# labgem/pangenomeNEM

Hardware: AMD Instinct MI355X
Metric: em_family_x_organism_cells_per_sec (higher is better)
Workload: dtype f32 chains with f64 intermediates (reference arithmetic); int32 popcounts in the M-step; 1 GPU; BASELINE configs[1]: 20000 families x 500 organisms, K=3, beta=0.5, contiguity graph (path + 5% chords, weights 1..8), ncem/sk_/pk; U-shaped family-frequency spectrum (Beta(0.3, 0.3) per family), default .m init; families_total=20000, families_per_gpu=20000, organisms=500, K=3, parallelism=1 GPU

## Files before the change

### pangenomenem_amd/csrc/nem_engine.hip

```cpp
#include <hip/hip_runtime.h>
#include <dlfcn.h>
#include <pthread.h>
#include <unistd.h>

#include <algorithm>
#include <atomic>
#include <cfloat>
#include <chrono>
#include <cmath>
#include <cstdio>
#include <cstdlib>
#include <cstring>
#include <condition_variable>
#include <deque>
#include <functional>
#include <map>
#include <string>
#include <mutex>
#include <thread>
#include <vector>

#include "nem_internal.hpp"
#include "nem_ff.hpp"
#include "nem_chain.hpp"
// ... 59 lines not shown
    void* rccl_comm = nullptr;
    int sh_world = 1, sh_rank = 0, sh_blk = 0, sh_stride = 0;
    const uint8_t* shard_lab[3] = {nullptr, nullptr, nullptr};
    int sh_tot_off() const { return ((sh_blk + 3) & ~3) + 4; }
    int npad = 0, dpad = 0, W = 0, wf = 0, nw64 = 0, device = 0;
    hipStream_t stream = nullptr;
    bool own_stream = false;
    nemgpu_config cfg{};
    bool have_matrix = false, have_params = false, has_graph = false;
    bool reset_pending = false;

    uint32_t* xw = nullptr;
    uint32_t* xws = nullptr;
    int* perm = nullptr;
    uint32_t* host_bits = nullptr; size_t host_bits_words = 0, host_bits_pin = 0;
    std::vector<uint32_t> host_bits_own;
    struct Staged { char* p; size_t size; };
    std::vector<Staged> staging;
    bool use_sort = true;
    uint64_t* xt = nullptr;
    int *nei_ptr = nullptr, *nei_idx = nullptr;
    float* nei_w = nullptr;
    int nnz = 0;

    float *prop = nullptr, *center = nullptr, *disp = nullptr;
    float *prop0 = nullptr, *center0 = nullptr, *disp0 = nullptr;
    size_t par_o_center = 0, par_o_disp = 0, par_o_nb = 0, par_words = 0;
    float *nbobs_k = nullptr, *iner = nullptr;
    int *fz_lastz = nullptr, *fz_any1 = nullptr;
    float *fz_in0 = nullptr, *fz_in1 = nullptr, *fz_inh = nullptr;
    float* fz_ct = nullptr;
    float* fz_chk = nullptr;
    double2* tabT = nullptr;
    double* tabL0 = nullptr;
    uint32_t *nz0 = nullptr, *nz1 = nullptr, *am0 = nullptr, *am1 = nullptr;
    double2* uni = nullptr;
    int* nonuni = nullptr;
    uint2* ffq = nullptr;
    int* sweep_next = nullptr;
    bool tables_fresh = false;
    bool density_fresh = false;
    double* pk = nullptr;
    float* logpk = nullptr;
    double* pkfki = nullptr;
    float* logpkfki = nullptr;

// ... 502 lines not shown

int do_density(nemgpu_engine* e)
{
    launch_density(finish_args(e, 0, nullptr), e->xws, e->n, e->npad, e->pkfki, e->logpkfki, e->iter_flags() + FLAG_MOVED,
                   kSweepFlagWords, e->stream);
    HIPCHK(hipGetLastError());
    e->flags_clean = true;
    e->density_fresh = true;
    return NEMGPU_OK;
}

struct SweepCtx {
    SweepArgs a{};
    bool use_nei = false;
    bool multi = false;
    int r = 0;
    int checked = 0;
    int slot_base = 0;
    bool post = false; bool post_moved = false; CtrlArgs post_ctrl{};
    SweepArgs* hold = nullptr;
    int* count_into = nullptr;
};

int clear_sweep_flags(nemgpu_engine* e)
{
    if (current_recorder()) launch_fill(e->iter_flags() + FLAG_MOVED, kSweepFlagWords, 0, e->stream);
    else HIPCHK(hipMemsetAsync(e->iter_flags() + FLAG_MOVED, 0, kSweepFlagWords * sizeof(int), e->stream));
    e->flags_clean = true;
    return NEMGPU_OK;
}

int ensure_draw_window(nemgpu_engine* e, long lo, long count)
{
    if (e->draw_valid && e->draw_tab0 <= lo && lo + count <= e->draw_tab0 + e->draw_cap) return NEMGPU_OK;
    if (e->draw_borrowed) {
        e->draw_borrowed = false; e->draw_valid = false; e->draw_tab = nullptr; e->draw_cap = 0;
    }
    long cap = std::max<long>(e->draw_cap, 1024);
    while (cap < 2 * count) cap *= 2;
    if (!e->draw_valid || lo < e->draw_tab0) {
        e->draw_gen.seed(e->cfg.tie_seed); e->draw_gen_pos = 0; e->draw_host.clear(); e->draw_tab0 = 0;
    }
    const long have_end = e->draw_tab0 + (long)e->draw_host.size();
    if (lo >= have_end) {
        while (e->draw_gen_pos < lo) { (void)e->draw_gen.next(); e->draw_gen_pos++; }
        e->draw_host.clear();
// ... 76 lines not shown
                continue;
            }
        } else if (c.post && ncem && r0 == 0 && b == count - 1) {
            c.a.post_on = 1; c.a.post_from_guess = (r % 2 == 1) ? 1 : 0; c.a.post_moved = c.post_moved ? 1 : 0;
            c.a.post_skip_guess = c.a.post_from_guess;
            c.a.post_nw64 = e->nw64; c.a.post_mask = e->mask; c.a.post_flags = e->iter_flags(); c.a.post_ctrl = c.post_ctrl;
        }
        launch_sweep(c.a, ncem, e->stream);
    }
    HIPCHK(hipGetLastError());
    return NEMGPU_OK;
}

int sweep_setup(nemgpu_engine* e, float beta, SweepCtx& c, bool id_by_value)
{
    c.use_nei = e->has_graph && beta != 0.0f;
    c.multi = c.use_nei || e->libc();
    SweepArgs& a = c.a;
    a.n_local = e->n; a.lo = e->lo; a.n_total = e->n_total; a.K = e->k; a.npad = e->npad;
    a.use_nei = c.use_nei ? 1 : 0;
    a.nei_ptr = e->nei_ptr; a.nei_idx = e->nei_idx; a.nei_w = e->nei_w;
    a.beta = beta;
    a.pkfki = e->pkfki;
    a.tie_rule = e->cfg.tie_rule; a.tie_seed = e->cfg.tie_seed; a.sweep_id = e->sweep_counter++;
    a.sweep_id_ptr = (e->stop_ptr != nullptr && !id_by_value) ? e->sweep_next : nullptr;
    if (e->libc()) {
        if (e->stop_ptr == nullptr) { int r = ensure_draw_window(e, e->draws, draw_need(e)); if (r) return r; }
        sweep_draw_args(e, a, e->stop_ptr == nullptr);
    }
    return NEMGPU_OK;
}

int sweep_enqueue(nemgpu_engine* e, float beta, SweepCtx& c, bool id_by_value = false, const CtrlArgs* post_ctrl = nullptr,
                  bool post_moved = false, int slot_base = 0, int rounds = 0, SweepArgs* hold = nullptr, int* count_into = nullptr)
{
    c = SweepCtx();
    c.slot_base = slot_base;
    if (post_ctrl != nullptr && e->ncem()) {
        c.post = true; c.post_moved = post_moved; c.post_ctrl = *post_ctrl; c.hold = hold;
        c.count_into = hold != nullptr ? count_into : nullptr;
    }
    { int r = sweep_setup(e, beta, c, id_by_value); if (r) return r; }
    if (!e->flags_clean) { int r = clear_sweep_flags(e); if (r) return r; }
    e->flags_clean = false;
    return sweep_launch_rounds(e, c, c.multi ? (rounds > 0 ? rounds : e->round_batch) : 1);
}
// ... 119 lines not shown
    if (e->ncem()) return do_labels_post(e, newbuf, oldbuf, ctrl);
    if (e->cfg.cvtest == NEMGPU_CV_CLAS) {
        launch_conv_fuzzy((size_t)e->n * e->k, e->cbuf[newbuf] + (size_t)e->lo * e->k,
                          e->cbuf[oldbuf] + (size_t)e->lo * e->k, e->cfg.cvthres, e->iter_flags(), e->stop_ptr, ctrl,
                          e->stream);
        HIPCHK(hipGetLastError());
    } else if (ctrl != nullptr) {
        launch_ctrl(*ctrl, e->stream);
        HIPCHK(hipGetLastError());
    }
    return NEMGPU_OK;
}

constexpr int kPipeDepth = 7;

int host_rounds_ctx(nemgpu_engine* e, SweepCtx& sc, uint32_t sweep_id, int launched)
{
    sc = SweepCtx();
    sc.use_nei = e->has_graph && e->cfg.beta != 0.0f;
    sc.multi = true;
    SweepArgs& a = sc.a;
    a.n_local = e->n; a.lo = e->lo; a.n_total = e->n_total; a.K = e->k; a.npad = e->npad; a.use_nei = sc.use_nei ? 1 : 0;
    a.nei_ptr = e->nei_ptr; a.nei_idx = e->nei_idx; a.nei_w = e->nei_w; a.beta = e->cfg.beta; a.pkfki = e->pkfki;
    a.tie_rule = e->cfg.tie_rule; a.tie_seed = e->cfg.tie_seed; a.sweep_id = sweep_id; a.sweep_id_ptr = nullptr;
    sc.r = launched; sc.checked = launched;
    if (e->libc()) {
        for (int q = 0; q < launched; q++) if (e->h_round(q)[FLAG_NTIES] & (1 << 30)) e->tie_heavy = true;
        int r = ensure_draw_window(e, e->draws, draw_need(e));
        if (r) return r;
        sweep_draw_args(e, a, true);
    }
    return NEMGPU_OK;
}

int iteration_rounds(const nemgpu_engine* e, int pos, bool deep)
{
    int want = (current_recorder() != nullptr || deep || !e->ncem()) ? e->round_batch : e->rounds_iter;
    if (!e->ncem() && current_recorder() == nullptr && pos >= 0 && pos < kFzPositions && e->fz_need[pos] > want) want = e->fz_need[pos];
    return want;
}

int enqueue_iteration(nemgpu_engine* e, int cur, uint32_t sweep_id, bool defer_ctrl, bool deep, int pos = -1)
{
    int r;
    const int saved = e->cur;
    e->cur = cur;
// ... 1285 lines not shown
    HIPCHK(hipSetDevice(device));
    nemgpu_engine* e = new nemgpu_engine();
    e->n_total = n_total; e->n_true = n_total; e->d = d; e->k = k; e->lo = site_lo; e->hi = site_hi; e->n = site_hi - site_lo;
    e->device = device;
    e->npad = (e->n + 255) / 256 * 256;
    e->dpad = (d + 63) / 64 * 64;
    e->W = e->dpad / 32;
    e->wf = (d + 31) / 32;
    e->nw64 = (e->n + 63) / 64;
    e->cfg.algo = NEMGPU_ALGO_NCEM; e->cfg.beta = 0.5f; e->cfg.disper = NEMGPU_DISP_K_; e->cfg.propor = NEMGPU_PROP_K;
    e->cfg.cvtest = NEMGPU_CV_CLAS; e->cfg.cvthres = 1e-8f; e->cfg.it_max = 100; e->cfg.param_fix = 0;
    e->cfg.tie_rule = NEMGPU_TIE_HASH; e->cfg.tie_seed = 0;
    if (const char* g = getenv("NEM_MI355X_GRAPHS")) e->use_graphs = (g[0] != '0');
    if (const char* g = getenv("NEM_MI355X_SHADOW_VERIFY")) e->shadow_verify = (g[0] != '0');
    e->flag_sets = e->shadow_verify ? 3 : 1;
    if (const char* g = getenv("NEM_MI355X_ROUND_COUNTS")) e->round_counts = (g[0] != '0');
    if (const char* g = getenv("NEM_MI355X_START_FUSED")) e->start_fused = (g[0] != '0');
    if (const char* g = getenv("NEM_MI355X_ROUNDS")) e->round_batch = std::max(2, std::min(kRoundBatchMax, atoi(g)));
    if (const char* g = getenv("NEM_MI355X_ROUNDS_ITER")) e->rounds_iter = std::max(2, std::min(e->round_batch, atoi(g)));
    e->rounds_iter = std::min(e->rounds_iter, e->round_batch);
    if (const char* g = getenv("NEM_MI355X_FAULT_INJECT")) e->fault_inject = !strcmp(g, "fuzzy_pc") ? 1 : 0;
    if (const char* g = getenv("NEM_MI355X_FF")) e->ff_mode = (g[0] == '0') ? 0 : (g[0] == '1') ? 1 : -1;
    if (const char* g = getenv("NEM_MI355X_SORT")) e->use_sort = (g[0] != '0');
    if (hip_stream) { e->stream = (hipStream_t)hip_stream; e->own_stream = false; }
    else {
        if (pool_stream_get(device, &e->stream) != hipSuccess) { delete e; set_error("hipStreamCreate failed"); return NEMGPU_E_DEVICE; }
        e->own_stream = true;
    }
    int r = NEMGPU_OK;
    alloc_for(e);
    auto A = [&](int rr) { if (r == NEMGPU_OK) r = rr; };
    A(dev_alloc(&e->xw, (size_t)e->W * e->npad));
    A(dev_alloc(&e->xws, (size_t)((e->W + 3) / 4) * 4 * e->npad));
    A(dev_alloc(&e->perm, (size_t)e->npad));
    A(dev_alloc(&e->xt, (size_t)d * e->nw64));
    A(alloc_model_buffers(e));
    if (r == NEMGPU_OK && !e->flags_host &&
        pool_get(device, true, e->flag_words() * sizeof(int), (char**)&e->flags_host, &e->flags_host_size) != hipSuccess) {
        set_error("hipHostMalloc failed"); r = NEMGPU_E_DEVICE;
    }
    if (r != NEMGPU_OK) { nemgpu_destroy(e); return r; }
    e->draw_ctl = e->sweep_next + 8;
    *out = e;
    return NEMGPU_OK;
}

// ... 233 lines not shown
    {
        std::vector<std::thread> th;
        for (int t = 1; t < nt; t++)
            th.emplace_back(pack_rows, (int)((long long)e->n * t / nt), (int)((long long)e->n * (t + 1) / nt), &badv[t]);
        pack_rows(0, (int)((long long)e->n / nt), &badv[0]);
        for (std::thread& x : th) x.join();
    }
    g_packers.fetch_sub(1);
    const uint64_t bad = badv[0] | badv[1] | badv[2] | badv[3];
    if (bad & 0xFEFEFEFEFEFEFEFEull) { e->host_bits_words = 0; set_error("presence/absence matrix must hold 0/1 only"); return NEMGPU_E_ARG; }
    return upload_bits(e, pc.data());
}

int nemgpu_set_graph(nemgpu_engine* e, const int32_t* ptr, const int32_t* idx, const float* w)
{
    if (!e || !ptr) return NEMGPU_E_FUNCARG;
    HIPCHK(hipSetDevice(e->device));
    const int nnz = ptr[e->n] - ptr[0];
    if (ptr[0] != 0 || nnz < 0) { set_error("graph: ptr[0] must be 0 and ptr non-decreasing"); return NEMGPU_E_ARG; }
    for (int i = 0; i < e->n; i++) if (ptr[i + 1] < ptr[i]) { set_error("graph: ptr not monotone"); return NEMGPU_E_ARG; }
    for (int t = 0; t < nnz; t++)
        if (idx[t] < 0 || idx[t] >= e->n_total) { set_error("graph: neighbour index out of range"); return NEMGPU_E_ARG; }
    e->nei_ptr = nullptr; e->nei_idx = nullptr; e->nei_w = nullptr;
    int r;
    alloc_for(e);
    const size_t b_ptr = sizeof(int) * ((size_t)e->n + 1), b_nz = sizeof(int) * (size_t)nnz;
    const size_t o_idx = (b_ptr + 255) & ~(size_t)255, o_w = (o_idx + b_nz + 255) & ~(size_t)255, total = o_w + b_nz;
    char* dev = nullptr;
    if ((r = dev_alloc(&dev, total))) return r;
    e->nei_ptr = (int*)dev; e->nei_idx = (int*)(dev + o_idx); e->nei_w = (float*)(dev + o_w);
    char* st = stage(e, total);
    if (st) {
        memcpy(st, ptr, b_ptr);
        if (nnz > 0) { memcpy(st + o_idx, idx, b_nz); memcpy(st + o_w, w, b_nz); }
        HIPCHK(hipMemcpyAsync(dev, st, total, hipMemcpyHostToDevice, e->stream));
    } else {
        HIPCHK(hipMemcpyAsync(e->nei_ptr, ptr, b_ptr, hipMemcpyHostToDevice, e->stream));
        if (nnz > 0) {
            HIPCHK(hipMemcpyAsync(e->nei_idx, idx, b_nz, hipMemcpyHostToDevice, e->stream));
            HIPCHK(hipMemcpyAsync(e->nei_w, w, b_nz, hipMemcpyHostToDevice, e->stream));
        }
        HIPCHK(hipStreamSynchronize(e->stream));
    }
    e->nnz = nnz;
    e->has_graph = nnz > 0;
    drop_graphs(e);
    return NEMGPU_OK;
}

int nemgpu_set_params(nemgpu_engine* e, const float* prop, const float* center, const float* disp)
{
    if (!e || !prop || !center || !disp) return NEMGPU_E_FUNCARG;
    HIPCHK(hipSetDevice(e->device));
    const size_t kd = (size_t)e->k * e->d;
    float* st = e->parent == nullptr ? (float*)stage(e, sizeof(float) * e->par_words) : nullptr;
    if (st) {
        memset(st, 0, sizeof(float) * e->par_words);
        memcpy(st, prop, sizeof(float) * e->k); memcpy(st + e->par_o_center, center, sizeof(float) * kd);
        memcpy(st + e->par_o_disp, disp, sizeof(float) * kd);
        HIPCHK(hipMemcpyAsync(e->prop0, st, sizeof(float) * e->par_words, hipMemcpyHostToDevice, e->stream));
    } else {
        HIPCHK(copy_sync(e, e->prop0, prop, sizeof(float) * e->k, hipMemcpyHostToDevice));
        HIPCHK(copy_sync(e, e->center0, center, sizeof(float) * kd, hipMemcpyHostToDevice));
        HIPCHK(copy_sync(e, e->disp0, disp, sizeof(float) * kd, hipMemcpyHostToDevice));
    }
    e->have_params = true;
    return reset_state(e, true);
}

int nemgpu_configure(nemgpu_engine* e, const nemgpu_config* cfg)
// ... 843 lines not shown
    if (m->block) (void)hipFree(m->block);
    delete m;
}

static int adopt_chunk(nemgpu_engine* e, const nemgpu_master* M, const nemk::ChunkPlan& plan, int nnz_c)
{
    if (e->device != M->device) { set_error("a chunk's engine lives on its master's device"); return NEMGPU_E_ARG; }
    HIPCHK(hipSetDevice(e->device));
    alloc_for(e);
    int r;
    const size_t words = (size_t)e->n * e->wf;
    if ((r = dev_alloc(&e->xf_stage, words + (size_t)e->npad))) return r;
    e->perm = reinterpret_cast<int*>(e->xf_stage + words);
    const int nnz = std::max(nnz_c, 0);
    const size_t b_ptr = sizeof(int) * ((size_t)e->n + 1), b_nz = sizeof(int) * (size_t)std::max(nnz, 1);
    const size_t o_idx = (b_ptr + 255) & ~(size_t)255, o_w = (o_idx + b_nz + 255) & ~(size_t)255, total = o_w + b_nz;
    char* dev = nullptr;
    if ((r = dev_alloc(&dev, total))) return r;
    e->nei_ptr = (int*)dev; e->nei_idx = (int*)(dev + o_idx); e->nei_w = (float*)(dev + o_w);
    nemk::ChunkFill f{e->n, e->d, e->wf, e->npad, e->xf_stage, e->perm, e->nei_ptr, e->nei_idx, e->nei_w};
    nemk::launch_chunk_fill(M->dev, plan, f, e->stream);
    HIPCHK(hipGetLastError());
    e->nnz = nnz; e->has_graph = nnz > 0;
    e->host_bits = nullptr; e->host_bits_words = 0;
    if (e->defer_layout) e->layout_pending = true;
    else { launch_layout(e->xf_stage, e->n, e->wf, e->W, e->npad, e->d, e->nw64, e->xw, e->xt, e->perm, e->xws, e->stream); HIPCHK(hipGetLastError()); }
    e->have_matrix = true;
    return NEMGPU_OK;
}

static int solve_chunks_impl(nemgpu_master* M, nemgpu_chunk* chunks, int count, int k, const float* prop, const float* center_k,
                             const float* disp_k, const nemgpu_config* cfg, int workers, int group, nemgpu_votes* votes,
                             ResampleTally* tally = nullptr)
{
    if (!M || !chunks || count <= 0 || k <= 0 || k > kMaxKernelK || !prop || !center_k || !disp_k || !cfg) return NEMGPU_E_FUNCARG;
    HIPCHK(hipSetDevice(M->device));
    const int n = M->n, nw64 = M->nw64, wf = M->wf, nnz = M->nnz;
    size_t org_total = 0;
    int max_dc = 0;
    for (int c = 0; c < count; c++) {
        nemgpu_chunk& q = chunks[c];
        q.rc = NEMGPU_OK; q.n = 0; q.nnz = 0; q.result = nemgpu_result{};
        if (!q.organisms || q.dc <= 0 || q.dc > M->d) { set_error("nemgpu_solve_chunks: chunk " + std::to_string(c) + ": 1 .. d organisms are needed"); return NEMGPU_E_FUNCARG; }
        for (int t = 0; t < q.dc; t++)
            if (q.organisms[t] < 0 || q.organisms[t] >= M->d) { set_error("nemgpu_solve_chunks: chunk " + std::to_string(c) + ": organism index out of range"); return NEMGPU_E_ARG; }
        org_total += ((size_t)q.dc + 63) & ~(size_t)63;
// ... 592 lines not shown
        e->masks_valid = false; e->tables_fresh = false; e->density_fresh = false;
        if ((r = do_mstep(e)) || (!e->ncem() && (r = read_iter_flags(e)))) { cleanup(); return r; }
        e->status = NEMGPU_OK; e->emptyk = 0;
        e->iters = best_res.iters; e->converged = best_res.converged;
        if (res) { *res = best_res; res->status = NEMGPU_OK; res->tie_draws = e->draws; for (int t = 0; t < 6; t++) res->crit[t] = best_crit[t]; }
    } else if (res) {
        fill_result(e, res);
        res->status = last_status;
    }
    if (best_start) *best_start = best;
    cleanup();
    return NEMGPU_OK;
}

static int make_clone(nemgpu_engine* p, nemgpu_engine** out, char* slab, size_t slab_bytes, int* flags_host, float* par0)
{
    nemgpu_engine* c = new nemgpu_engine();
    c->n_total = p->n_total; c->n_true = p->n_true; c->d = p->d; c->k = p->k; c->lo = p->lo; c->hi = p->hi; c->n = p->n;
    c->npad = p->npad; c->dpad = p->dpad; c->W = p->W; c->wf = p->wf; c->nw64 = p->nw64; c->device = p->device;
    c->stream = p->stream; c->own_stream = false;
    c->cfg = p->cfg; c->have_matrix = true; c->have_params = true; c->has_graph = p->has_graph;
    c->xw = p->xw; c->xws = p->xws; c->perm = p->perm; c->xt = p->xt; c->use_sort = p->use_sort;
    c->nei_ptr = p->nei_ptr; c->nei_idx = p->nei_idx; c->nei_w = p->nei_w; c->nnz = p->nnz;
    c->use_graphs = p->use_graphs; c->ff_mode = p->ff_mode; c->round_batch = p->round_batch; c->rounds_iter = p->rounds_iter;
    c->parent = p; c->carve_all = true;
    c->chunks.push_back({slab, slab_bytes, 0, false});
    c->shared_chunk = 0;
    c->flags_host = flags_host; c->flags_host_borrowed = true;
    const size_t kd = (size_t)p->k * p->d;
    c->prop0 = par0; c->center0 = par0 + p->k; c->disp0 = par0 + p->k + kd;
    alloc_for(c);
    int r = alloc_model_buffers(c);
    if (r == NEMGPU_OK) r = ensure_state_buffers(c);
    if (r == NEMGPU_OK) r = ensure_crit_buffers(c);
    alloc_for(p);
    if (r != NEMGPU_OK) { nemgpu_destroy(c); return r; }
    c->draw_ctl = c->sweep_next + 8;
    *out = c;
    return NEMGPU_OK;
}

static int ensure_clones(nemgpu_engine* e, int count)
{
    if ((int)e->clones.size() >= count) return NEMGPU_OK;
    HIPCHK(hipStreamSynchronize(e->stream));
    for (nemgpu_engine* c : e->clones) nemgpu_destroy(c);
// ... 351 lines not shown

int nemgpu_stats_words(const nemgpu_engine* e) { return e ? e->k + e->k * e->d : 0; }

int nemgpu_shard_layout(nemgpu_engine* e, int world, int rank, int blk, int stride, int n_true)
{
    if (!e || world <= 0 || rank < 0 || rank >= world || blk <= 0 || stride < blk + 1 || n_true <= 0) return NEMGPU_E_FUNCARG;
    if (e->lo != rank * stride || e->n > blk || e->n_total != world * stride) {
        set_error("shard layout does not match the engine's slot range");
        return NEMGPU_E_ARG;
    }
    if (stride % 4 != 0) { set_error("shard layout: stride must be a multiple of 4 bytes"); return NEMGPU_E_ARG; }
    e->sh_world = world; e->sh_rank = rank; e->sh_blk = blk; e->sh_stride = stride; e->n_true = n_true;
    return NEMGPU_OK;
}

namespace {
void shard_sweep_args(nemgpu_engine* e, SweepArgs& a, float beta, int sweep_id)
{
    a = SweepArgs{};
    a.n_local = e->n; a.lo = e->lo; a.n_total = e->n_total; a.K = e->k; a.npad = e->npad;
    a.use_nei = (e->has_graph && beta != 0.0f) ? 1 : 0;
    a.nei_ptr = e->nei_ptr; a.nei_idx = e->nei_idx; a.nei_w = e->nei_w;
    a.beta = beta; a.pkfki = e->pkfki;
    a.tie_rule = e->cfg.tie_rule; a.tie_seed = e->cfg.tie_seed;
    a.sweep_id = sweep_id >= 0 ? (uint32_t)sweep_id : 0u;
    a.sweep_id_ptr = sweep_id >= 0 ? nullptr : e->sweep_next;
    a.stop = e->stop_ptr;
    a.n_ranks = e->sh_world; a.slot_stride = e->sh_stride; a.slot_pad = e->sh_stride - e->sh_blk;
    a.fold_ticket = e->sweep_next + 32;
    if (e->libc()) { sweep_draw_args(e, a, e->stop_ptr == nullptr); a.rank_index = e->sh_rank; }
}
uint8_t* own_flag_byte(nemgpu_engine* e, uint8_t* labels) { return labels + (size_t)e->sh_rank * e->sh_stride + e->sh_blk; }
int shard_buf(const nemgpu_engine* e, const uint8_t* p) { for (int b = 0; b < 3; b++) if (e->shard_lab[b] == p) return b; return -1; }
int shard_tie_args(nemgpu_engine* e, SweepArgs& a, const uint8_t* guess, uint8_t* out)
{
    if (!e->libc()) return NEMGPU_OK;
    const int g = shard_buf(e, guess), o = shard_buf(e, out);
    if (g < 0 || o < 0) { set_error("TIE_LIBC in the sharded path: a label array that nemgpu_shard_set_labels was not told about"); return NEMGPU_E_FUNCARG; }
    a.tie_cnt_guess = e->tie_cnt[g]; a.tie_cnt_out = e->tie_cnt[o];
    a.rank_tot_in = guess + e->sh_tot_off();
    a.rank_tot_out = out + (size_t)e->sh_rank * e->sh_stride + e->sh_tot_off();
    return NEMGPU_OK;
}
void shard_round1_args(nemgpu_engine* e, SweepArgs& a, float beta, int sweep_id, const uint8_t* labels_old_dev,
                       const uint8_t* labels_guess_dev, uint8_t* labels_out_dev)
{
// ... 974 lines not shown
```

### pangenomenem_amd/csrc/nem_kernels.hpp

```cpp
#pragma once
#include <hip/hip_runtime.h>
#include <cstdint>
#include <cstring>
#include <type_traits>
#include <vector>

#include "../../include/nem_mi355x.h"

namespace nemk {

constexpr int kMaxKernelK = 32;
constexpr int kTicketWords = 32 * 33;
constexpr double kEpsilonD = 1e-20;

enum { FLAG_CHANGED = 0, FLAG_NZERO = 1, FLAG_FIRSTZERO = 2, FLAG_NTIES = 3, FLAG_ROUND_STRIDE = 4 };
enum { FLAG_EMPTYK = 0, FLAG_EMPTY_PROP = 1, FLAG_FAULT = 2, FLAG_MOVED = 3, FLAG_ITER_STRIDE = 4 };

enum { C_STOP = 0, C_FOLD = 1, C_ITERS = 10, C_COMMITS = 2, C_STATUS = 3, C_EMPTYK = 4, C_CONVERGED = 5, C_NEED_ROUNDS = 6,
       C_SWEEP_ROUNDS = 7, C_NZERO = 8, C_FIRSTZERO = 9, C_DRAWS = 11, C_DEEP = 12, C_DRAWS_INIT = 13, C_INIT_ROUNDS = 14, C_WORDS = 16 };

struct CtrlArgs {
    int* ctrl; const int* iter_flags; const int* round0;
    int n_rounds;
    int param_fix, use_nei, cvtest, ncem; float cvthres;
// ... 14 lines not shown
    const int* nei_ptr; const int* nei_idx; const float* nei_w;
    float beta;
    const double* pkfki;
    const uint8_t* lab_old; const uint8_t* lab_guess; uint8_t* lab_out;
    const float* c_old; const float* c_guess; float* c_out;
    int tie_rule; uint32_t tie_seed; uint32_t sweep_id;
    const int* sweep_id_ptr;
    int* flags;
    const int* prev_changed;
    const int* stop;
    const uint8_t* flags_in; int n_ranks, slot_stride, slot_pad;
    int post_on, post_from_guess, post_moved, post_nw64, post_skip_guess;
    int post_no_masks;
    uint64_t* post_mask; int* post_flags;
    CtrlArgs post_ctrl;
    uint8_t* publish_byte; int* publish_ticket;
    int* fold_ticket;
    const uint32_t* draw_tab; int draw_tab_len, draw_base, draw_tab0;
    const int* draw_ctl; const int* draw_extra;
    const int* tie_cnt_guess; int* tie_cnt_out;
    const uint8_t* rank_tot_in; int rank_index; uint8_t* rank_tot_out;
    int spb;
    int* post_stats; const uint64_t* post_xt; int post_D;
};
struct LabelsPostArgs { int n_local, lo, K, nw64; const uint8_t* lab_new; const uint8_t* lab_old; uint64_t* mask; int* flags;
                        const int* stop; CtrlArgs ca; };
struct CountsArgs { int K, D, nw64; const uint64_t* xt; const uint64_t* mask; int* stats; const int* stop; CtrlArgs prev_ctrl; };
struct FuzzyArgs { int n, npad, K, D; const uint32_t* xw; const uint64_t* xt; int nw64; const float* c; float* nbobs_k;
                   float* in0; float* in1; float* inh_k; int* lastz; int* any1; float* center; float* iner; const int* stop;
                   float* ct; int ctpad;
                   float* chk;
                   int* fault;
                   int inject; };
struct ConvFuzzyArgs { size_t m; const float* c; const float* cold; float thres; int* flags; const int* stop; CtrlArgs ca; };
struct OnehotArgs { int n, K; const uint8_t* lab; float* c; };
struct CritArgs { int n, K, npad; const int* nei_ptr; const int* nei_idx; const float* nei_w; int use_nei; float beta;
                  const float* c; const double* pkfki; const float* logpkfki; float* dik; float* gik; double* lfi; double* lzi;
                  float* crit6; int hard; };
struct FillArgs { int* ptr; int words; int value; };
struct CopyArgs { const int* src; int* dst; int words; };
struct CopySegsArgs { const int* src[8]; int* dst[8]; int words[8]; int n; };
void launch_copy_segments(const CopySegsArgs& a, hipStream_t s);
struct LayoutArgs { const uint32_t* xf; const int* perm; int n, wf, W, npad, d, nw64; uint32_t* xw; uint32_t* xws; uint64_t* xt; };

enum OpKind { OP_FINISH = 1, OP_DENSITY, OP_DENSITY_FUSED, OP_SWEEP, OP_COUNTS, OP_LABELS_POST, OP_CTRL,
              OP_CONV_FUZZY, OP_ONEHOT, OP_CRIT_TERMS, OP_CRIT_REDUCE, OP_CRIT_FINAL, OP_FILL, OP_COPY, OP_FUZZY_T,
              OP_FUZZY_PC, OP_FUZZY_MED2, OP_LAYOUT_WORDS, OP_LAYOUT_BITS };
// ... 91 lines not shown
```

### pangenomenem_amd/csrc/nem_sweep.hip

```cpp
#include <hip/hip_runtime.h>
#include <algorithm>
#include <cstdio>
#include <cstdlib>

#include "nem_kernels.hpp"
#include "nem_sweep_dev.hpp"

namespace nemk {

template <int KT, bool NCEM, int BS, bool LIBC = false, bool COUNT = false>
__global__ __launch_bounds__(BS) void k_sweep(SweepArgs a) { sweep_body<KT, NCEM, BS, LIBC, COUNT>(a, blockIdx.x, gridDim.x); }
template <int KT, bool NCEM, int BS, bool LIBC = false>
__global__ __launch_bounds__(BS) void k_sweep_b(const void* arr, int stride, const int* gx) { NEM_B_HEAD(SweepArgs) sweep_body<KT, NCEM, BS, LIBC>(a, blockIdx.x, nblk); }

static int sweep_variant(int K, bool ncem, bool big, bool libc) { return (K >= 1 && K <= 10 ? K : 0) | (ncem ? 16 : 0) | (big ? 32 : 0) | (libc && ncem ? 64 : 0); }

template <bool BATCHED>
static void sweep_dispatch(int variant, dim3 grid, unsigned bdim, hipStream_t s, const SweepArgs* a, const void* arr, int stride, const int* gx)
{
    const int kt = variant & 15; const bool ncem = (variant & 16) != 0, big = (variant & 32) != 0, libc = (variant & 64) != 0;
    dim3 block(bdim);
#define NEM_SW2(KT_, NC_, BS_, LC_)                                                                                \
    do {                                                                                                           \
        if (BATCHED) hipLaunchKernelGGL((k_sweep_b<KT_, NC_, BS_, LC_>), grid, block, 0, s, arr, stride, gx);     \
        else hipLaunchKernelGGL((k_sweep<KT_, NC_, BS_, LC_>), grid, block, 0, s, *a);                             \
    } while (0)
#define NEM_SW(KT_)                                                                                                \
    case KT_:                                                                                                      \
        if (big) { if (!ncem) NEM_SW2(KT_, false, 1024, false); else if (libc) NEM_SW2(KT_, true, 1024, true); else NEM_SW2(KT_, true, 1024, false); } \
        else { if (!ncem) NEM_SW2(KT_, false, 256, false); else if (libc) NEM_SW2(KT_, true, 256, true); else NEM_SW2(KT_, true, 256, false); }       \
        break;
    switch (kt) {
        NEM_SW(1) NEM_SW(2) NEM_SW(3) NEM_SW(4) NEM_SW(5) NEM_SW(6) NEM_SW(7) NEM_SW(8) NEM_SW(9) NEM_SW(10)
    default:
        if (!ncem) NEM_SW2(0, false, 256, false); else if (libc) NEM_SW2(0, true, 256, true); else NEM_SW2(0, true, 256, false);
    }
// ... 49 lines not shown
```

### pangenomenem_amd/csrc/nem_sweep_dev.hpp

```cpp
#pragma once
#include <hip/hip_runtime.h>
#include <cstdint>

#include "nem_kernels.hpp"

namespace nemk {

__host__ __device__ inline uint32_t mix32(uint32_t seed, uint32_t sweep, uint32_t site)
{
    uint32_t h = seed * 0x9E3779B1u + sweep * 0x85EBCA77u + site * 0xC2B2AE3Du + 0x27D4EB2Fu;
    h ^= h >> 16; h *= 0x7FEB352Du;
    h ^= h >> 15; h *= 0x846CA68Bu;
    h ^= h >> 16;
    return h;
}

__device__ inline void ctrl_logic(const CtrlArgs& a)
{
    int* c = a.ctrl;
    constexpr int kMaxRounds = 8;
    const int nr = a.n_rounds > 0 ? (a.n_rounds < kMaxRounds ? a.n_rounds : kMaxRounds) : 2;
    const int stop = c[C_STOP];
    int iters = c[C_ITERS], commits = c[C_COMMITS], sweep_rounds = c[C_SWEEP_ROUNDS], nzero = c[C_NZERO], firstzero = c[C_FIRSTZERO];
    int draws = c[C_DRAWS];
// ... 195 lines not shown
        return false;
    }
    const float u = (float)(1.0 / K);
#pragma unroll
    for (int k = 0; k < KA; k++) if (k < K) cf[k] = u;
    return true;
}

constexpr int kLabMask = 0x7F, kLabDrew = 0x80;
constexpr int kTabShort = 1 << 30;
constexpr int kInnerCap = 64;

__device__ __forceinline__ int wave_sum_i32(int v)
{
    v += __builtin_amdgcn_update_dpp(0, v, 0xB1, 0xF, 0xF, false);
    v += __builtin_amdgcn_update_dpp(0, v, 0x4E, 0xF, 0xF, false);
    v += __builtin_amdgcn_update_dpp(0, v, 0x141, 0xF, 0xF, false);
    v += __builtin_amdgcn_update_dpp(0, v, 0x140, 0xF, 0xF, false);
    v += __builtin_amdgcn_update_dpp(0, v, 0x142, 0xA, 0xF, false);
    v += __builtin_amdgcn_update_dpp(0, v, 0x143, 0xC, 0xF, false);
    return __builtin_amdgcn_readlane(v, 63);
}

template <int KT, bool NCEM, int BS, bool LIBC = false, bool COUNT = false>
__device__ __forceinline__ void sweep_body(const SweepArgs& a, const int bx, const int nblk)
{
    static_assert(!COUNT || (NCEM && BS == 256 && !LIBC && KT > 0), "the counting round: NCEM, 256 sites per block");
    int fold_hint = 0;
    if (a.stop != nullptr) {
        static_assert(C_STOP == 0 && C_FOLD == 1, "one 8-byte load");
        const int2 sf = *reinterpret_cast<const int2*>(a.stop);
        if (sf.x) return;
        fold_hint = sf.y;
    }
    bool skip = (a.prev_changed != nullptr && *a.prev_changed == 0);
    if (a.flags_in != nullptr) {
        int any = 0;
        for (int r = 0; r < a.n_ranks; r++) any |= a.flags_in[(size_t)r * a.slot_stride];
        if (!any) skip = true;
    }
    if (skip && !(NCEM && a.post_on)) {
        if (a.publish_byte != nullptr && bx == 0 && threadIdx.x == 0) *a.publish_byte = 0;
        if (LIBC && a.prev_changed != nullptr && bx == 0 && threadIdx.x == 0) a.flags[FLAG_NTIES] = a.prev_changed[FLAG_NTIES - FLAG_CHANGED];
        return;
    }
    __shared__ int s_nzero, s_first;
    __shared__ int s_chg, s_mov;
    constexpr int kExpTab = 64;
    __shared__ double s_exp[NCEM ? kExpTab : 1];
    __shared__ __attribute__((aligned(16))) uint8_t s_lab[NCEM ? BS : 1];
    __shared__ uint64_t s_drew[BS / 64];
    const int spb = (BS > 256 && a.spb > 0) ? a.spb : BS;
    const int i = bx * spb + threadIdx.x;
    const bool active = (int)threadIdx.x < spb && i < a.n_local;
    const int gi = a.lo + (active ? i : 0);
    const int K = KT > 0 ? KT : a.K;
    constexpr int KA = KT > 0 ? KT : kMaxKernelK;
    bool zero_density = false;
    bool changed = false;
    int my_guess = 0, my_old = 0, my_new = 255;
    if (NCEM && active) { my_guess = a.lab_guess[gi]; my_old = a.lab_old[gi] & kLabMask; }
    int blk_cnt_guess = 0;
    if (LIBC && threadIdx.x == 0 && a.tie_cnt_guess != nullptr) blk_cnt_guess = a.tie_cnt_guess[bx];
    constexpr int kCntRows = COUNT ? kFusedMaxD / BS : 1;
    uint64_t xs[kCntRows][4];
    if (COUNT) {
        const int w0 = 4 * bx;
#pragma unroll
        for (int q = 0; q < kCntRows; q++) {
            const int d = (int)threadIdx.x + q * BS;
#pragma unroll
            for (int w = 0; w < 4; w++)
                xs[q][w] = (d < a.post_D && w0 + w < a.post_nw64) ? a.post_xt[(size_t)d * a.post_nw64 + w0 + w] : 0ull;
        }
    }
    __shared__ int s_anydrew;
    if (threadIdx.x == 0) { s_nzero = 0; s_first = 0; s_chg = 0; s_mov = 0; s_anydrew = 0; }
    if (NCEM) s_lab[threadIdx.x] = (uint8_t)my_guess;
    if (NCEM && a.use_nei && !skip && threadIdx.x < kExpTab) s_exp[threadIdx.x] = exp((double)a.beta * (double)(float)threadIdx.x);
    __shared__ int s_lower;
    if (LIBC && !skip && threadIdx.x < 64 && a.tie_cnt_guess != nullptr) {
        int part = 0;
        for (int b = threadIdx.x; b < bx; b += 64) part += a.tie_cnt_guess[b];
        part = wave_sum_i32(part);
        if (threadIdx.x == 0) {
            if (a.rank_tot_in != nullptr)
                for (int r = 0; r < a.rank_index; r++) part += *reinterpret_cast<const int*>(a.rank_tot_in + (size_t)r * a.slot_stride);
            s_lower = part;
        }
    }
    bool blk_drew = false;
    if (LIBC) blk_drew = __syncthreads_or((my_guess & kLabDrew) != 0) != 0;
    else __syncthreads();

    if (NCEM) {
    constexpr bool libc = LIBC;
    const int blk_lo = a.lo + bx * spb;
    double pkf[KA];
#pragma unroll
    for (int k = 0; k < KA; k++) if (k < K) pkf[k] = active && !skip ? a.pkfki[(size_t)k * a.npad + i] : 0.0;
    int nb = 0, ne = 0;
    int dyn[4]; float wn[4]; int fl[4];
#pragma unroll
    for (int u = 0; u < 4; u++) { dyn[u] = -1; wn[u] = 0.0f; fl[u] = 255; }
    if (active && !skip && a.use_nei) {
        nb = a.nei_ptr[i]; ne = a.nei_ptr[i + 1];
        int jn[4];
#pragma unroll
        for (int u = 0; u < 4; u++) {
            const bool ok = nb + u < ne;
            jn[u] = ok ? a.nei_idx[nb + u] : gi;
            wn[u] = ok ? a.nei_w[nb + u] : 0.0f;
        }
#pragma unroll
        for (int u = 0; u < 4; u++) {
            if (nb + u < ne) {
                if (jn[u] < gi && jn[u] >= blk_lo) dyn[u] = jn[u] - blk_lo;
                else fl[u] = ((jn[u] < gi) ? a.lab_guess[jn[u]] : a.lab_old[jn[u]]) & kLabMask;
            }
        }
    }
    const bool long_row = ne - nb > 4;
    int lower_draws = -1;
    bool tab_short = false;
    int cur = my_guess;
    int seen[4] = {-1, -1, -1, -1};
    uint64_t seen_drew = ~0ull; int seen_wave_draws = -1;
    for (int it = 0; it < kInnerCap; it++) {
        int below_in_block = 0;
        uint64_t drew_lt = 0;
        if (libc && blk_drew) {
            const uint64_t bal = __ballot((s_lab[threadIdx.x] & kLabDrew) != 0);
            if ((threadIdx.x & 63) == 0) s_drew[threadIdx.x >> 6] = bal;
            __syncthreads();
            for (int w = 0; w < (int)(threadIdx.x >> 6); w++) below_in_block += (int)__popcll(s_drew[w]);
            drew_lt = s_drew[threadIdx.x >> 6] & ((1ull << (threadIdx.x & 63)) - 1ull);
        }
        int nxt = cur;
        if (active && !skip) {
            int lab[4];
            bool same = it != 0 && !long_row;
#pragma unroll
            for (int u = 0; u < 4; u++) {
                lab[u] = dyn[u] >= 0 ? (s_lab[dyn[u]] & kLabMask) : fl[u];
                same = same && (dyn[u] < 0 || lab[u] == seen[u]);
            }
            if (libc) same = same && drew_lt == seen_drew && below_in_block == seen_wave_draws;
            if (!same) {
                float ctx[KA];
#pragma unroll
                for (int k = 0; k < KA; k++) ctx[k] = 0.0f;
#pragma unroll
                for (int u = 0; u < 4; u++) {
                    seen[u] = lab[u];
                    if (nb + u < ne) {
#pragma unroll
                        for (int k = 0; k < KA; k++)
                            if (k < K) ctx[k] = ctx[k] + ((lab[u] == k) ? wn[u] : -0.0f);
                    }
                }
                for (int t = nb + 4; t < ne; t++) {
                    const int j = a.nei_idx[t];
                    const float wt = a.nei_w[t];
                    int l;
                    if (j < gi && j >= blk_lo) l = s_lab[j - blk_lo] & kLabMask;
                    else l = ((j < gi) ? a.lab_guess[j] : a.lab_old[j]) & kLabMask;
#pragma unroll
                    for (int k = 0; k < KA; k++)
                        if (k < K) ctx[k] = ctx[k] + ((l == k) ? wt : -0.0f);
                }
                float cf[KA];
                zero_density = local_proba<KA>(a, K, pkf, ctx, cf, s_exp, kExpTab);
                int kmax = 0; float ukmax = cf[0];
#pragma unroll
                for (int k = 1; k < KA; k++) if (k < K && cf[k] > ukmax) { ukmax = cf[k]; kmax = k; }
                int drew = 0;
                if (a.tie_rule != NEMGPU_TIE_FIRST) {
                    int nequal = 0;
// ... 150 lines not shown
        if ((int)threadIdx.x < K) {
            const int k = threadIdx.x;
            const int v = __popcll(s_cmask[k][0]) + __popcll(s_cmask[k][1]) + __popcll(s_cmask[k][2]) + __popcll(s_cmask[k][3]);
            if (v != 0) atomicAdd(&st[k], v);
        }
    }
    const bool post_ctrl = NCEM && a.post_on && a.post_ctrl.ctrl != nullptr;
    if (a.publish_byte != nullptr || post_ctrl || fold) {
        int* ticket = a.publish_byte != nullptr ? a.publish_ticket : (post_ctrl ? a.post_ctrl.ticket : a.fold_ticket);
        if (last_block_ticket(ticket, nblk, fold ? s_nzero : 0, fold ? &a.flags[FLAG_NZERO] : nullptr, bx)) {
            if (a.publish_byte != nullptr) {
                *a.publish_byte = (uint8_t)(__hip_atomic_load(&a.flags[FLAG_CHANGED], __ATOMIC_RELAXED, __HIP_MEMORY_SCOPE_AGENT) != 0);
                if (NCEM && a.post_on && a.post_moved)
                    a.publish_byte[1] = (uint8_t)(__hip_atomic_load(&a.post_flags[FLAG_MOVED], __ATOMIC_RELAXED, __HIP_MEMORY_SCOPE_AGENT) != 0);
                if (LIBC && a.rank_tot_out != nullptr)
                    *reinterpret_cast<int*>(a.rank_tot_out) =
                        __hip_atomic_load(&a.flags[FLAG_NTIES], __ATOMIC_RELAXED, __HIP_MEMORY_SCOPE_AGENT) & (kTabShort - 1);
            }
            if (post_ctrl) ctrl_logic(a.post_ctrl);
        }
    }
}

}
```

Before: 343.3 billion cells/s.

## Pack first four neighbours per site and hoist sweep head loads

Adds a prepass kernel that packs each site's first four neighbour indices and weights into int4/float4 arrays. The NCEM sweep kernel now issues all per-site loads up front (stop flags, labels, pkfki, packed neighbours, neighbour labels) before the shared-memory setup and barriers. Inline asm pins these values in registers so the loads overlap rather than running as dependent scattered accesses. The cost is extra device memory, higher register pressure that may reduce occupancy, and pkfki and neighbour loads that now happen even for skipped sites.

```diff
diff --git a/pangenomenem_amd/csrc/nem_engine.hip b/pangenomenem_amd/csrc/nem_engine.hip
--- a/pangenomenem_amd/csrc/nem_engine.hip
+++ b/pangenomenem_amd/csrc/nem_engine.hip
@@ -105,6 +105,9 @@
     int *nei_ptr = nullptr, *nei_idx = nullptr;
     float* nei_w = nullptr;
     int nnz = 0;
+    int4* nei_i4 = nullptr;
+    float4* nei_w4 = nullptr;
+    bool sweep_head = true;
 
     float *prop = nullptr, *center = nullptr, *disp = nullptr;
     float *prop0 = nullptr, *center0 = nullptr, *disp0 = nullptr;
@@ -653,6 +656,19 @@
     int* count_into = nullptr;
 };
 
+int build_graph_head(nemgpu_engine* e)
+{
+    e->nei_i4 = nullptr; e->nei_w4 = nullptr;
+    if (!e->sweep_head || e->nnz <= 0 || e->dry_run) return NEMGPU_OK;
+    int r;
+    alloc_for(e);
+    if ((r = dev_alloc(&e->nei_i4, (size_t)e->n)) || (r = dev_alloc(&e->nei_w4, (size_t)e->n))) { e->nei_i4 = nullptr; e->nei_w4 = nullptr; return r; }
+    nemk::launch_graph_head(e->n, e->nei_ptr, e->nei_idx, e->nei_w, e->nei_i4, e->nei_w4, e->stream);
+    HIPCHK(hipGetLastError());
+    return NEMGPU_OK;
+}
+void sweep_head_args(const nemgpu_engine* e, SweepArgs& a) { a.nei_i4 = e->nei_i4; a.nei_w4 = e->nei_w4; }
+
 int clear_sweep_flags(nemgpu_engine* e)
 {
     if (current_recorder()) launch_fill(e->iter_flags() + FLAG_MOVED, kSweepFlagWords, 0, e->stream);
@@ -775,6 +791,7 @@
     a.nei_ptr = e->nei_ptr; a.nei_idx = e->nei_idx; a.nei_w = e->nei_w;
     a.beta = beta;
     a.pkfki = e->pkfki;
+    if (e->ncem()) sweep_head_args(e, a);
     a.tie_rule = e->cfg.tie_rule; a.tie_seed = e->cfg.tie_seed; a.sweep_id = e->sweep_counter++;
     a.sweep_id_ptr = (e->stop_ptr != nullptr && !id_by_value) ? e->sweep_next : nullptr;
     if (e->libc()) {
@@ -940,6 +957,7 @@
     SweepArgs& a = sc.a;
     a.n_local = e->n; a.lo = e->lo; a.n_total = e->n_total; a.K = e->k; a.npad = e->npad; a.use_nei = sc.use_nei ? 1 : 0;
     a.nei_ptr = e->nei_ptr; a.nei_idx = e->nei_idx; a.nei_w = e->nei_w; a.beta = e->cfg.beta; a.pkfki = e->pkfki;
+    if (e->ncem()) sweep_head_args(e, a);
     a.tie_rule = e->cfg.tie_rule; a.tie_seed = e->cfg.tie_seed; a.sweep_id = sweep_id; a.sweep_id_ptr = nullptr;
     sc.r = launched; sc.checked = launched;
     if (e->libc()) {
@@ -2271,6 +2289,7 @@
     if (const char* g = getenv("NEM_MI355X_FAULT_INJECT")) e->fault_inject = !strcmp(g, "fuzzy_pc") ? 1 : 0;
     if (const char* g = getenv("NEM_MI355X_FF")) e->ff_mode = (g[0] == '0') ? 0 : (g[0] == '1') ? 1 : -1;
     if (const char* g = getenv("NEM_MI355X_SORT")) e->use_sort = (g[0] != '0');
+    if (const char* g = getenv("NEM_MI355X_SWEEP_HEAD")) e->sweep_head = (g[0] != '0');
     if (hip_stream) { e->stream = (hipStream_t)hip_stream; e->own_stream = false; }
     else {
         if (pool_stream_get(device, &e->stream) != hipSuccess) { delete e; set_error("hipStreamCreate failed"); return NEMGPU_E_DEVICE; }
@@ -2550,6 +2569,7 @@
     for (int t = 0; t < nnz; t++)
         if (idx[t] < 0 || idx[t] >= e->n_total) { set_error("graph: neighbour index out of range"); return NEMGPU_E_ARG; }
     e->nei_ptr = nullptr; e->nei_idx = nullptr; e->nei_w = nullptr;
+    e->nei_i4 = nullptr; e->nei_w4 = nullptr;
     int r;
     alloc_for(e);
     const size_t b_ptr = sizeof(int) * ((size_t)e->n + 1), b_nz = sizeof(int) * (size_t)nnz;
@@ -2573,7 +2593,7 @@
     e->nnz = nnz;
     e->has_graph = nnz > 0;
     drop_graphs(e);
-    return NEMGPU_OK;
+    return build_graph_head(e);
 }
 
 int nemgpu_set_params(nemgpu_engine* e, const float* prop, const float* center, const float* disp)
@@ -3463,6 +3483,7 @@
     nemk::launch_chunk_fill(M->dev, plan, f, e->stream);
     HIPCHK(hipGetLastError());
     e->nnz = nnz; e->has_graph = nnz > 0;
+    if ((r = build_graph_head(e))) return r;
     e->host_bits = nullptr; e->host_bits_words = 0;
     if (e->defer_layout) e->layout_pending = true;
     else { launch_layout(e->xf_stage, e->n, e->wf, e->W, e->npad, e->d, e->nw64, e->xw, e->xt, e->perm, e->xws, e->stream); HIPCHK(hipGetLastError()); }
@@ -4101,6 +4122,7 @@
     c->cfg = p->cfg; c->have_matrix = true; c->have_params = true; c->has_graph = p->has_graph;
     c->xw = p->xw; c->xws = p->xws; c->perm = p->perm; c->xt = p->xt; c->use_sort = p->use_sort;
     c->nei_ptr = p->nei_ptr; c->nei_idx = p->nei_idx; c->nei_w = p->nei_w; c->nnz = p->nnz;
+    c->nei_i4 = p->nei_i4; c->nei_w4 = p->nei_w4; c->sweep_head = p->sweep_head;
     c->use_graphs = p->use_graphs; c->ff_mode = p->ff_mode; c->round_batch = p->round_batch; c->rounds_iter = p->rounds_iter;
     c->parent = p; c->carve_all = true;
     c->chunks.push_back({slab, slab_bytes, 0, false});
@@ -4498,6 +4520,7 @@
     a.use_nei = (e->has_graph && beta != 0.0f) ? 1 : 0;
     a.nei_ptr = e->nei_ptr; a.nei_idx = e->nei_idx; a.nei_w = e->nei_w;
     a.beta = beta; a.pkfki = e->pkfki;
+    sweep_head_args(e, a);
     a.tie_rule = e->cfg.tie_rule; a.tie_seed = e->cfg.tie_seed;
     a.sweep_id = sweep_id >= 0 ? (uint32_t)sweep_id : 0u;
     a.sweep_id_ptr = sweep_id >= 0 ? nullptr : e->sweep_next;
diff --git a/pangenomenem_amd/csrc/nem_kernels.hpp b/pangenomenem_amd/csrc/nem_kernels.hpp
--- a/pangenomenem_amd/csrc/nem_kernels.hpp
+++ b/pangenomenem_amd/csrc/nem_kernels.hpp
@@ -60,7 +60,10 @@
     const uint8_t* rank_tot_in; int rank_index; uint8_t* rank_tot_out;
     int spb;
     int* post_stats; const uint64_t* post_xt; int post_D;
+    const int4* nei_i4; const float4* nei_w4;
 };
+void launch_graph_head(int n, const int* ptr, const int* idx, const float* w, int4* i4, float4* w4, hipStream_t s);
+
 struct LabelsPostArgs { int n_local, lo, K, nw64; const uint8_t* lab_new; const uint8_t* lab_old; uint64_t* mask; int* flags;
                         const int* stop; CtrlArgs ca; };
 struct CountsArgs { int K, D, nw64; const uint64_t* xt; const uint64_t* mask; int* stats; const int* stop; CtrlArgs prev_ctrl; };
diff --git a/pangenomenem_amd/csrc/nem_sweep.hip b/pangenomenem_amd/csrc/nem_sweep.hip
--- a/pangenomenem_amd/csrc/nem_sweep.hip
+++ b/pangenomenem_amd/csrc/nem_sweep.hip
@@ -12,6 +12,23 @@
 __global__ __launch_bounds__(BS) void k_sweep(SweepArgs a) { sweep_body<KT, NCEM, BS, LIBC, COUNT>(a, blockIdx.x, gridDim.x); }
 template <int KT, bool NCEM, int BS, bool LIBC = false>
 __global__ __launch_bounds__(BS) void k_sweep_b(const void* arr, int stride, const int* gx) { NEM_B_HEAD(SweepArgs) sweep_body<KT, NCEM, BS, LIBC>(a, blockIdx.x, nblk); }
+
+__global__ __launch_bounds__(256) void k_graph_head(int n, const int* __restrict__ ptr, const int* __restrict__ idx,
+                                                    const float* __restrict__ w, int4* __restrict__ i4, float4* __restrict__ w4)
+{
+    const int i = blockIdx.x * 256 + threadIdx.x;
+    if (i >= n) return;
+    const int b = ptr[i], e = ptr[i + 1];
+    int j[4]; float v[4];
+#pragma unroll
+    for (int u = 0; u < 4; u++) { const bool ok = b + u < e; j[u] = ok ? idx[b + u] : -1; v[u] = ok ? w[b + u] : 0.0f; }
+    i4[i] = make_int4(j[0], j[1], j[2], j[3]);
+    w4[i] = make_float4(v[0], v[1], v[2], v[3]);
+}
+void launch_graph_head(int n, const int* ptr, const int* idx, const float* w, int4* i4, float4* w4, hipStream_t s)
+{
+    if (n > 0) hipLaunchKernelGGL(k_graph_head, dim3((n + 255) / 256), dim3(256), 0, s, n, ptr, idx, w, i4, w4);
+}
 
 static int sweep_variant(int K, bool ncem, bool big, bool libc) { return (K >= 1 && K <= 10 ? K : 0) | (ncem ? 16 : 0) | (big ? 32 : 0) | (libc && ncem ? 64 : 0); }
 
diff --git a/pangenomenem_amd/csrc/nem_sweep_dev.hpp b/pangenomenem_amd/csrc/nem_sweep_dev.hpp
--- a/pangenomenem_amd/csrc/nem_sweep_dev.hpp
+++ b/pangenomenem_amd/csrc/nem_sweep_dev.hpp
@@ -241,18 +241,97 @@
     return __builtin_amdgcn_readlane(v, 63);
 }
 
+#define NEM_SWEEP_NEI_REGS \
+    if (NCEM && active && !skip && a.use_nei) { \
+        int jn[4]; \
+        if (head) { \
+             \
+            nb = nb_h; ne = ne_h; \
+            int raw[4]; \
+            _Pragma("unroll") \
+            for (int u = 0; u < 4; u++) { \
+                jn[u] = jn_h[u]; wn[u] = wn_h[u]; has[u] = jn[u] >= 0; \
+                const bool local = jn[u] < gi && jn[u] >= blk_lo; \
+                const int j = (has[u] && !local) ? jn[u] : gi; \
+                raw[u] = ((j < gi) ? a.lab_guess : a.lab_old)[j]; \
+            } \
+            _Pragma("unroll") \
+            for (int u = 0; u < 4; u++) { \
+                if (has[u]) { \
+                    if (jn[u] < gi && jn[u] >= blk_lo) dyn[u] = jn[u] - blk_lo; \
+                    else fl[u] = raw[u] & kLabMask; \
+                } \
+            } \
+        } else { \
+            nb = a.nei_ptr[i]; ne = a.nei_ptr[i + 1]; \
+            _Pragma("unroll") \
+            for (int u = 0; u < 4; u++) { \
+                has[u] = nb + u < ne; \
+                jn[u] = has[u] ? a.nei_idx[nb + u] : gi; \
+                wn[u] = has[u] ? a.nei_w[nb + u] : 0.0f; \
+            } \
+            _Pragma("unroll") \
+            for (int u = 0; u < 4; u++) { \
+                if (has[u]) { \
+                    if (jn[u] < gi && jn[u] >= blk_lo) dyn[u] = jn[u] - blk_lo; \
+                    else fl[u] = ((jn[u] < gi) ? a.lab_guess[jn[u]] : a.lab_old[jn[u]]) & kLabMask; \
+                } \
+            } \
+        } \
+    }
+
 template <int KT, bool NCEM, int BS, bool LIBC = false, bool COUNT = false>
 __device__ __forceinline__ void sweep_body(const SweepArgs& a, const int bx, const int nblk)
 {
     static_assert(!COUNT || (NCEM && BS == 256 && !LIBC && KT > 0), "the counting round: NCEM, 256 sites per block");
+    constexpr bool kHeadFits = !(LIBC && BS > 256 && KT == 8);
+    const bool head = NCEM && kHeadFits && a.nei_i4 != nullptr;
+    const int spb = (BS > 256 && a.spb > 0) ? a.spb : BS;
+    const int i = bx * spb + threadIdx.x;
+    const bool active = (int)threadIdx.x < spb && i < a.n_local;
+    const int gi = a.lo + (active ? i : 0);
+    const int K = KT > 0 ? KT : a.K;
+    constexpr int KA = KT > 0 ? KT : kMaxKernelK;
+    int my_guess = 0, my_old = 0, my_new = 255;
+    double pkf_h[KA];
+    int nb_h = 0, ne_h = 0;
+    int jn_h[4] = {-1, -1, -1, -1}; float wn_h[4] = {0.0f, 0.0f, 0.0f, 0.0f};
+    int2 sf_h = make_int2(0, 0); int pc_h = 1;
+    if (head) {
+        static_assert(C_STOP == 0 && C_FOLD == 1, "one 8-byte load");
+        if (a.stop != nullptr) sf_h = *reinterpret_cast<const int2*>(a.stop);
+        if (a.prev_changed != nullptr) pc_h = *a.prev_changed;
+        if (active) { my_guess = a.lab_guess[gi]; my_old = a.lab_old[gi]; }
+#pragma unroll
+        for (int k = 0; k < KA; k++) pkf_h[k] = (k < K && active) ? a.pkfki[(size_t)k * a.npad + i] : 0.0;
+        if (active && a.use_nei) {
+            nb_h = a.nei_ptr[i]; ne_h = a.nei_ptr[i + 1];
+            const int4 j4 = a.nei_i4[i]; const float4 w4 = a.nei_w4[i];
+            jn_h[0] = j4.x; jn_h[1] = j4.y; jn_h[2] = j4.z; jn_h[3] = j4.w;
+            wn_h[0] = w4.x; wn_h[1] = w4.y; wn_h[2] = w4.z; wn_h[3] = w4.w;
+        }
+    }
     int fold_hint = 0;
-    if (a.stop != nullptr) {
-        static_assert(C_STOP == 0 && C_FOLD == 1, "one 8-byte load");
-        const int2 sf = *reinterpret_cast<const int2*>(a.stop);
-        if (sf.x) return;
-        fold_hint = sf.y;
-    }
-    bool skip = (a.prev_changed != nullptr && *a.prev_changed == 0);
+    bool skip;
+    if (head) {
+        asm volatile("" : "+v"(my_guess), "+v"(my_old), "+v"(nb_h), "+v"(ne_h));
+#pragma unroll
+        for (int u = 0; u < 4; u++) asm volatile("" : "+v"(jn_h[u]), "+v"(wn_h[u]));
+#pragma unroll
+        for (int k = 0; k < KA; k++) asm volatile("" : "+v"(pkf_h[k]));
+        my_old &= kLabMask;
+        if (sf_h.x) return;
+        fold_hint = sf_h.y;
+        skip = pc_h == 0;
+    } else {
+        if (a.stop != nullptr) {
+            static_assert(C_STOP == 0 && C_FOLD == 1, "one 8-byte load");
+            const int2 sf = *reinterpret_cast<const int2*>(a.stop);
+            if (sf.x) return;
+            fold_hint = sf.y;
+        }
+        skip = (a.prev_changed != nullptr && *a.prev_changed == 0);
+    }
     if (a.flags_in != nullptr) {
         int any = 0;
         for (int r = 0; r < a.n_ranks; r++) any |= a.flags_in[(size_t)r * a.slot_stride];
@@ -269,16 +348,9 @@
     __shared__ double s_exp[NCEM ? kExpTab : 1];
     __shared__ __attribute__((aligned(16))) uint8_t s_lab[NCEM ? BS : 1];
     __shared__ uint64_t s_drew[BS / 64];
-    const int spb = (BS > 256 && a.spb > 0) ? a.spb : BS;
-    const int i = bx * spb + threadIdx.x;
-    const bool active = (int)threadIdx.x < spb && i < a.n_local;
-    const int gi = a.lo + (active ? i : 0);
-    const int K = KT > 0 ? KT : a.K;
-    constexpr int KA = KT > 0 ? KT : kMaxKernelK;
     bool zero_density = false;
     bool changed = false;
-    int my_guess = 0, my_old = 0, my_new = 255;
-    if (NCEM && active) { my_guess = a.lab_guess[gi]; my_old = a.lab_old[gi] & kLabMask; }
+    if (NCEM && active && !head) { my_guess = a.lab_guess[gi]; my_old = a.lab_old[gi] & kLabMask; }
     int blk_cnt_guess = 0;
     if (LIBC && threadIdx.x == 0 && a.tie_cnt_guess != nullptr) blk_cnt_guess = a.tie_cnt_guess[bx];
     constexpr int kCntRows = COUNT ? kFusedMaxD / BS : 1;
@@ -293,6 +365,12 @@
                 xs[q][w] = (d < a.post_D && w0 + w < a.post_nw64) ? a.post_xt[(size_t)d * a.post_nw64 + w0 + w] : 0ull;
         }
     }
+    int nb = 0, ne = 0;
+    int dyn[4]; float wn[4]; int fl[4]; bool has[4];
+#pragma unroll
+    for (int u = 0; u < 4; u++) { dyn[u] = -1; wn[u] = 0.0f; fl[u] = 255; has[u] = false; }
+    const int blk_lo = a.lo + bx * spb;
+    if (head) { NEM_SWEEP_NEI_REGS }
     __shared__ int s_anydrew;
     if (threadIdx.x == 0) { s_nzero = 0; s_first = 0; s_chg = 0; s_mov = 0; s_anydrew = 0; }
     if (NCEM) s_lab[threadIdx.x] = (uint8_t)my_guess;
@@ -314,31 +392,10 @@
 
     if (NCEM) {
     constexpr bool libc = LIBC;
-    const int blk_lo = a.lo + bx * spb;
     double pkf[KA];
 #pragma unroll
-    for (int k = 0; k < KA; k++) if (k < K) pkf[k] = active && !skip ? a.pkfki[(size_t)k * a.npad + i] : 0.0;
-    int nb = 0, ne = 0;
-    int dyn[4]; float wn[4]; int fl[4];
-#pragma unroll
-    for (int u = 0; u < 4; u++) { dyn[u] = -1; wn[u] = 0.0f; fl[u] = 255; }
-    if (active && !skip && a.use_nei) {
-        nb = a.nei_ptr[i]; ne = a.nei_ptr[i + 1];
-        int jn[4];
-#pragma unroll
-        for (int u = 0; u < 4; u++) {
-            const bool ok = nb + u < ne;
-            jn[u] = ok ? a.nei_idx[nb + u] : gi;
-            wn[u] = ok ? a.nei_w[nb + u] : 0.0f;
-        }
-#pragma unroll
-        for (int u = 0; u < 4; u++) {
-            if (nb + u < ne) {
-                if (jn[u] < gi && jn[u] >= blk_lo) dyn[u] = jn[u] - blk_lo;
-                else fl[u] = ((jn[u] < gi) ? a.lab_guess[jn[u]] : a.lab_old[jn[u]]) & kLabMask;
-            }
-        }
-    }
+    for (int k = 0; k < KA; k++) if (k < K) pkf[k] = head ? pkf_h[k] : (active && !skip ? a.pkfki[(size_t)k * a.npad + i] : 0.0);
+    if (!head) { NEM_SWEEP_NEI_REGS }
     const bool long_row = ne - nb > 4;
     int lower_draws = -1;
     bool tab_short = false;
@@ -372,7 +429,7 @@
 #pragma unroll
                 for (int u = 0; u < 4; u++) {
                     seen[u] = lab[u];
-                    if (nb + u < ne) {
+                    if (has[u]) {
 #pragma unroll
                         for (int k = 0; k < KA; k++)
                             if (k < K) ctx[k] = ctx[k] + ((lab[u] == k) ? wn[u] : -0.0f);
@@ -569,4 +626,6 @@
     }
 }
 
+#undef NEM_SWEEP_NEI_REGS
+
 }
```

Result: faster. 347.1 billion cells/s (median of 6 runs) (+1.1%).
